# Zhongxu-Wang/ArtSpeech

Measured on AMD Instinct MI355X. Metric: mel frames/sec (whole job; per-GPU = value / n_gpus), acoustic-model inference path, batch 32 x 200-frame utterances, higher is better.
Workload: dtype f32 (f16x3 split-operand MFMA, fp32 accumulate)

## Files before the change

### artspeech_amd/_lib.py

```python
import ctypes
import os

import torch

_HERE = os.path.dirname(os.path.abspath(__file__))
LIB_PATH = os.environ.get("AS_LIB_PATH") or os.path.join(_HERE, "lib", "libartspeech_hip.so")
_lib = None

c_p = ctypes.c_void_p
c_i = ctypes.c_int
c_sz = ctypes.c_size_t
c_f = ctypes.c_float

_SIGNATURES = {
    "as_abi_version": (c_i, []),
    "as_device_status": (c_i, [c_i]),
    "as_device_status_raise_for_test": (c_i, [c_i, c_p]),
    "as_set_range_probe": (c_i, [c_i]),
    "as_prof_enable": (c_i, [c_i]),
    "as_prof_collect": (c_i, [c_p, c_p, c_p, c_p, c_i]),
    "as_prof_hint": (c_i, [ctypes.c_double, ctypes.c_double]),
    "as_prof_bracket_overhead": (c_i, [c_p, c_p]),
    "as_prof_mfma_sustained": (c_i, [c_p, c_p, c_p]),
    "as_mas_workspace_bytes": (c_sz, [c_i, c_i, c_i]),
    "as_mas_f32": (c_i, [c_p, c_p, c_p, c_i, c_i, c_i, c_i, c_p, c_p, c_p, c_p, c_sz, c_p]),
    "as_softmax_mas_f32": (c_i, [c_p, c_p, c_p, c_i, c_i, c_i, c_i, c_i, c_p, c_p, c_p, c_p, c_p, c_sz, c_p]),
}

AS_MAX_TAPS = 25
AS_ABI_VERSION = 10
AS_PROSODY_DIM, AS_PROSODY_TRACKS, AS_PROSODY_DUR, AS_PROSODY_GAIN, AS_PROSODY_OFFSET = 25, 12, 0, 1, 13


class ConvGemmArgs(ctypes.Structure):
    _fields_ = [("Wh", ctypes.c_void_p), ("W", ctypes.c_void_p), ("X", ctypes.c_void_p), ("Xh", ctypes.c_void_p), ("Y", ctypes.c_void_p),
                ("Yh", ctypes.c_void_p), ("bias", ctypes.c_void_p), ("res", ctypes.c_void_p), ("meta", ctypes.c_void_p),
                ("ws", ctypes.c_void_p), ("ws_bytes", ctypes.c_size_t),
                ("M", ctypes.c_int32), ("N", ctypes.c_int32), ("K", ctypes.c_int32), ("T", ctypes.c_int32),
                ("Kp", ctypes.c_int32),
                ("ldx", ctypes.c_int32), ("ldy", ctypes.c_int32), ("ldr", ctypes.c_int32),
                ("act", ctypes.c_int32), ("div_sqrt2", ctypes.c_int32), ("in_act", ctypes.c_int32),
                ("transpose_out", ctypes.c_int32), ("yh_lrelu", ctypes.c_int32), ("n_prod", ctypes.c_int32),
                ("dh", ctypes.c_int32 * AS_MAX_TAPS), ("dw", ctypes.c_int32 * AS_MAX_TAPS),
                ("in_slope", ctypes.c_float), ("act_slope", ctypes.c_float), ("acc_scale", ctypes.c_float),
                ("n_groups", ctypes.c_int32), ("group_cols", ctypes.c_int32), ("range_probe", ctypes.c_int32), ("status", ctypes.c_void_p),
                ("Xh2", ctypes.c_void_p), ("K2", ctypes.c_int32), ("src_col", ctypes.c_void_p), ("N_in", ctypes.c_int32), ("ileave_u", ctypes.c_int32),
                ("slab_tr", ctypes.c_int32), ("n_valid", ctypes.c_void_p)]


_SIGNATURES.update({
    "as_make_meta": (c_i, [c_p, c_p, c_i, c_i, c_i, c_p, c_p]),
    "as_conv_gemm_f32": (c_i, [ctypes.POINTER(ConvGemmArgs), c_p]),
    "as_conv_gemm_workspace_bytes": (c_sz, [ctypes.POINTER(ConvGemmArgs)]),
    "as_conv_gemm_multi_f32": (c_i, [ctypes.POINTER(ConvGemmArgs), c_i, c_p]),
    "as_conv_gemm_multi_tile": (c_i, [ctypes.POINTER(ConvGemmArgs), c_i]),
    "as_conv_gemm_multi_workspace_bytes": (c_sz, [ctypes.POINTER(ConvGemmArgs)]),
    "as_conv_gemm_plan": (c_i, [ctypes.POINTER(ConvGemmArgs), ctypes.POINTER(ctypes.c_int32), ctypes.POINTER(ctypes.c_int32),
                                ctypes.POINTER(ctypes.c_int32)]),
    "as_split_f16x2_bytes": (c_sz, [c_i, c_i]),
    "as_split_f16x2_f32": (c_i, [c_p, c_i, c_i, c_i, c_i, c_f, c_p, c_p]),
    "as_prep_weight_f16x2_bytes": (c_sz, [c_i, c_i, c_i, c_i]),
    "as_prep_weight_f16x2_host": (c_i, [c_p, c_i, c_i, c_i, c_i, c_p, c_p]),
    "as_prep_weight_f16x2_sc_bytes": (c_sz, [c_i, c_i, c_i, c_i, c_i]),
    "as_prep_weight_f16x2_sc_host": (c_i, [c_p, c_p, c_i, c_i, c_i, c_i, c_i, c_p, c_p]),
    "as_embed_groups_f32": (c_i, [c_p, c_i, c_p, c_p, c_i, c_i, c_i, c_i, c_f, c_p, c_i, c_p]),
    "as_channel_layernorm_groups_f32": (c_i, [c_p, c_i, c_i, c_i, c_p, c_p, c_p, c_p, c_i, c_f, c_i, c_p, c_i, c_p]),
    "as_channel_layernorm_split_f32": (c_i, [c_p, c_i, c_i, c_i, c_p, c_p, c_p, c_p, c_i, c_f, c_i, c_p, c_p]),
    "as_relpos_attention_groups_f32": (c_i, [c_p, c_i, c_i, c_i, c_i, c_p, c_p, c_p, c_p, c_i, c_p, c_i, c_i, c_p, c_i, c_p]),
    "as_embed_f32": (c_i, [c_p, c_p, c_i, c_i, c_i, c_f, c_p, c_i, c_p]),
    "as_channel_layernorm_f32": (c_i, [c_p, c_i, c_i, c_i, c_p, c_p, c_f, c_i, c_p, c_i, c_p]),
    "as_adain_f32": (c_i, [c_p, c_i, c_i, c_p, c_i, c_p, c_i, c_p, c_i, c_i, c_p, c_p, c_p, c_i, c_p]),
    "as_adain_split_f32": (c_i, [c_p, c_i, c_i, c_p, c_i, c_p, c_i, c_i, c_i, c_p, c_p]),
    "as_linear_rows_f32": (c_i, [c_p, c_i, c_p, c_p, c_i, c_i, c_i, c_p, c_i, c_p]),
    "as_durations_f32": (c_i, [c_p, c_p, c_p, c_i, c_p, c_p, c_p, c_i, c_p]),
    "as_expand_f32": (c_i, [c_p, c_i, c_i, c_p, c_i, c_i, c_p, c_i, c_p]),
    "as_ref_features_f32": (c_i, [c_p, c_i, c_i, c_p, c_p, c_i, c_i, c_p, c_p, c_i, c_p]),
    "as_crop_f32": (c_i, [c_p, c_i, c_p, c_i, c_p, c_i, c_p, c_i, c_i, c_i, c_p]),
    "as_rows_to_images_f32": (c_i, [c_p, c_i, c_p, c_i, c_i, c_p, c_p, c_i, c_i, c_p]),
    "as_stem_pool_image_f32": (c_i, [c_p, c_p, c_p, c_i, c_p, c_p, c_i, c_i, c_p, c_i, c_p, c_i, c_i, c_i, c_i, c_p, c_i, c_p]),
    "as_dwconv_down_f32": (c_i, [c_p, c_i, c_p, c_p, c_i, c_p, c_i, c_p, c_p, c_i, c_p, c_p, c_i, c_i, c_i, c_i, c_i, c_p]),
    "as_frame_signal_f32": (c_i, [c_p, c_p, c_p, c_i, c_i, c_i, c_i, c_p, c_i, c_p]),
    "as_spec_power_f32": (c_i, [c_p, c_i, c_i, c_i, c_p, c_i, c_p]),
    "as_log_norm_f32": (c_i, [c_p, c_i, c_i, c_i, c_f, c_f, c_f, c_p, c_i, c_p]),
    "as_xl_attention_f32": (c_i, [c_p, c_i, c_i, c_i, c_p, c_i, c_p, c_p, c_f, c_p, c_i, c_i, c_p, c_i, c_p]),
    "as_glu_dwconv_bn_swish_f32": (c_i, [c_p, c_i, c_i, c_p, c_i, c_p, c_p, c_p, c_i, c_p, c_i, c_p]),
    "as_lstm_step0_f32": (c_i, [c_p, c_i, c_i, c_i, c_p, c_i, c_p]),
    "as_bn_lrelu_maxpool_rows_f32": (c_i, [c_p, c_i, c_p, c_i, c_i, c_i, c_i, c_p, c_p, c_f, c_p, c_i, c_i, c_i, c_p]),
    "as_avgpool_down_f32": (c_i, [c_p, c_i, c_p, c_p, c_i, c_p, c_i, c_p, c_p, c_i, c_i, c_p, c_i, c_i, c_i, c_i, c_p]),
    "as_im2col_valid_f32": (c_i, [c_p, c_i, c_p, c_p, c_i, c_p, c_i, c_p, c_p, c_i, c_i, c_i, c_i, c_i, c_i, c_i, c_p]),
    "as_dwconv_down_image_f32": (c_i, [c_p, c_i, c_p, c_p, c_i, c_p, c_p, c_i, c_p, c_p, c_i, c_i, c_i, c_i, c_i, c_p, c_i, c_p]),
    "as_avgpool_down_image_f32": (c_i, [c_p, c_i, c_p, c_p, c_i, c_p, c_i, c_p, c_p, c_i, c_i, c_p, c_i, c_i, c_i, c_i, c_p, c_i, c_i, c_p]),
    "as_im2col_valid_image_f32": (c_i, [c_p, c_i, c_p, c_p, c_p, c_p, c_i, c_i, c_i, c_i, c_i, c_p, c_p]),
    "as_mean_pool_f32": (c_i, [c_p, c_i, c_p, c_i, c_i, c_i, c_p, c_i, c_p]),
    "as_relpos_attention_f32": (c_i, [c_p, c_i, c_i, c_i, c_i, c_p, c_p, c_p, c_i, c_i, c_p, c_i, c_p]),
    "as_relpos_attention_image_f32": (c_i, [c_p, c_i, c_p, c_i, c_i, c_i, c_i, c_p, c_p, c_p, c_p, c_i, c_p, c_i, c_i, c_p, c_i, c_p, c_p]),
    "as_bilstm_f32": (c_i, [c_p, c_i, c_p, c_i, c_i, c_p]),
    "as_bilstm_cluster_bytes": (ctypes.c_size_t, [c_i, c_i]),
    "as_bilstm_cluster_f32": (c_i, [c_p, c_i, c_p, c_i, c_i, c_i, c_p, ctypes.c_size_t, c_p]),
    "as_interleave_phases_f32": (c_i, [c_p, c_i, c_p, c_i, c_i, c_i, c_p, c_i, c_p]),
    "as_mean3_f32": (c_i, [c_p, c_p, c_p, c_i, c_i, c_i, c_p, c_i, c_p]),
})


class LnArgs(ctypes.Structure):
    _fields_ = [("gamma", c_p), ("beta", c_p), ("gamma2", c_p), ("beta2", c_p), ("n_split", ctypes.c_int32), ("eps", ctypes.c_float),
                ("relu", ctypes.c_int32), ("yh", c_p)]


class AdainArgs(ctypes.Structure):
    _fields_ = [("x", c_p), ("ldx", ctypes.c_int32), ("C", ctypes.c_int32), ("gb", c_p), ("gb_off", c_p), ("ldgb", ctypes.c_int32),
                ("gb_sc", ctypes.c_int32), ("col_off", c_p), ("src_off", c_p), ("U", ctypes.c_int32), ("N", ctypes.c_int32),
                ("lrelu", ctypes.c_int32), ("yh", c_p), ("pool_w", c_p), ("pool_b", c_p), ("x_up", c_p), ("ld_up", ctypes.c_int32),
                ("col_w", c_p)]


class DownArgs(ctypes.Structure):
    _fields_ = [("kind", ctypes.c_int32), ("x", c_p), ("ldx", ctypes.c_int32), ("in_off", c_p), ("in_w", c_p), ("Hin", ctypes.c_int32),
                ("y", c_p), ("ldy", ctypes.c_int32), ("out_off", c_p), ("out_w", c_p), ("Hout", ctypes.c_int32), ("w", c_p), ("bias", c_p),
                ("kh", ctypes.c_int32), ("pool_h", ctypes.c_int32), ("Kp", ctypes.c_int32), ("res", c_p), ("ldr", ctypes.c_int32),
                ("B", ctypes.c_int32), ("C", ctypes.c_int32), ("max_out", ctypes.c_int32), ("lrelu", ctypes.c_int32), ("yh", c_p),
                ("n_out", ctypes.c_int32)]


class ResPairArgs(ctypes.Structure):
    _fields_ = [("x", c_p), ("ldx", ctypes.c_int32), ("y", c_p), ("ldy", ctypes.c_int32), ("w1", c_p), ("w2", c_p), ("b1", c_p), ("b2", c_p),
                ("scale1", ctypes.c_float), ("scale2", ctypes.c_float), ("C", ctypes.c_int32), ("N", ctypes.c_int32), ("k", ctypes.c_int32),
                ("dil", ctypes.c_int32), ("slope", ctypes.c_float), ("col_off", c_p), ("B", ctypes.c_int32), ("max_w", ctypes.c_int32),
                ("add1", c_p), ("add2", c_p), ("ld_add", ctypes.c_int32), ("out_div", ctypes.c_float), ("yh", c_p), ("yh_slope", ctypes.c_float),
                ("x_u", ctypes.c_int32), ("x_bias", c_p)]


class ModelCfg(ctypes.Structure):
    _fields_ = [("hidden_dim", ctypes.c_int32), ("dim_in", ctypes.c_int32), ("style_dim", ctypes.c_int32), ("n_mels", ctypes.c_int32),
                ("n_token", ctypes.c_int32), ("reserved", ctypes.c_int32), ("stats", ctypes.c_float * 24)]


class Batch(ctypes.Structure):
    _fields_ = [("B", ctypes.c_int32), ("tok_lens", ctypes.POINTER(ctypes.c_int32)), ("ref_lens", ctypes.POINTER(ctypes.c_int32)),
                ("frames", ctypes.POINTER(ctypes.c_int32))]


class ForwardIO(ctypes.Structure):
    _fields_ = [("tokens", c_p), ("mel", c_p), ("ld_mel", ctypes.c_int32), ("f0_raw", c_p), ("ema_raw", c_p), ("ld_ema", ctypes.c_int32),
                ("forced_dur", c_p), ("mel_out", c_p), ("ld_out", ctypes.c_int32), ("duration", c_p), ("dur_i", c_p), ("frame_off", c_p),
                ("style", c_p), ("feat12", c_p), ("ld_feat", ctypes.c_int32), ("t_en", c_p), ("a_en", c_p), ("ld_en", ctypes.c_int32),
                ("F0", c_p), ("N", c_p), ("EMA", c_p), ("ld_pred", ctypes.c_int32), ("frame_cap", ctypes.c_int32), ("segs", c_p),
                ("voices", c_p), ("ld_voice", ctypes.c_int32), ("n_voices", ctypes.c_int32), ("voice_idx", c_p),
                ("prosody", c_p), ("ld_prosody", ctypes.c_int32)]


class HostIO(ctypes.Structure):
    _fields_ = [("tokens", c_p), ("mel", c_p), ("ld_mel", ctypes.c_int32), ("f0_raw", c_p), ("ema_raw", c_p), ("ld_ema", ctypes.c_int32),
                ("forced_dur", c_p), ("mel_out", c_p), ("ld_out", ctypes.c_int32), ("frame_cap", ctypes.c_int32), ("frame_off", c_p),
                ("voices", c_p), ("ld_voice", ctypes.c_int32), ("n_voices", ctypes.c_int32), ("voice_idx", c_p),
                ("prosody", c_p), ("ld_prosody", ctypes.c_int32)]


class TokenProsody(ctypes.Structure):
    _fields_ = [("rows", c_p), ("ld", ctypes.c_int32), ("smooth", ctypes.c_int32)]


(AS_MOD_FORWARD_A, AS_MOD_FORWARD_B, AS_MOD_ENCODER, AS_MOD_STYLE, AS_MOD_DURATION, AS_MOD_ARTS, AS_MOD_DECODER, AS_MOD_FORWARD_B_CAP,
 AS_MOD_VOICE, AS_MOD_FORWARD_A_VOICE) = range(10)
_pB, _pIO = ctypes.POINTER(Batch), ctypes.POINTER(ForwardIO)
_SIGNATURES.update({
    "as_adain_image_f32": (c_i, [ctypes.POINTER(AdainArgs), c_p]),
    "as_conv_gemm_multi_post_f32": (c_i, [ctypes.POINTER(ConvGemmArgs), ctypes.POINTER(AdainArgs), ctypes.POINTER(ctypes.c_int32),
                                          ctypes.POINTER(LnArgs), c_i, c_p]),
    "as_down_multi_f32": (c_i, [ctypes.POINTER(DownArgs), c_i, c_p]),
    "as_down_strip_rule": (c_i, [c_i, c_i, c_i, c_i, c_i, ctypes.POINTER(ctypes.c_int32), ctypes.POINTER(ctypes.c_int32)]),
    "as_respair_f32": (c_i, [ctypes.POINTER(ResPairArgs), c_p]),
    "as_xl_attention_image_f32": (c_i, [c_p, c_i, c_p, c_p, c_i, c_i, c_i, ctypes.c_float, c_p, c_i, c_i, c_p, c_i, c_p, c_p]),
    "as_mean3_image_f32": (c_i, [c_p, c_p, c_p, c_i, c_i, c_i, ctypes.c_float, c_p, c_p]),
    "as_conv_post_f32": (c_i, [c_p, c_i, c_i, c_i, c_p, c_p, c_i, ctypes.c_float, c_i, c_p, c_p, c_p]),
    "as_rows_image_f32": (c_i, [c_p, c_i, c_i, c_i, c_p, c_p]),
    "as_project_cols_f32": (c_i, [c_p, c_i, c_i, c_i, c_p, c_p, c_i, c_p, c_i, c_p]),
    "as_pointwise_small_f32": (c_i, [c_p, c_i, c_i, c_i, c_p, c_p, c_i, c_p, c_i, c_p, c_p, c_i, c_p, c_p]),
    "as_model_create": (c_i, [c_p, c_sz, ctypes.POINTER(ModelCfg), ctypes.POINTER(c_p)]),
# ... 155 lines not shown
```

### artspeech_amd/csrc/attention.hip

```cpp
#include <cstring>
#include "common.h"
#include "artspeech_hip.h"
#define AS_FILE_CLS AS_CLS_ATTN

#define QT 16
#define KT 64
#define KPAD 65
#define MAXDK 128
#define MAXREL 9

static __device__ __forceinline__ float wmax(float v)
{
#pragma unroll
    for (int o = 32; o > 0; o >>= 1) v = fmaxf(v, __shfl_xor(v, o));
    return v;
}
static __device__ __forceinline__ float wsum(float v)
{
#pragma unroll
    for (int o = 32; o > 0; o >>= 1) v += __shfl_xor(v, o);
    return v;
}

__global__ void __launch_bounds__(256)
// ... 43 lines not shown
    float m[4], l[4], acc[4][2];
#pragma unroll
    for (int qq = 0; qq < 4; ++qq) { m[qq] = -INFINITY; l[qq] = 0.f; acc[qq][0] = 0.f; acc[qq][1] = 0.f; }
    float* Pw = Ps + wave * KT * 4;
    const int d0 = lane, d1 = lane + 64;

    for (int k0 = 0; k0 < N; k0 += KT) {
        __syncthreads();
        for (int i = tid; i < dk * KT; i += 256) {
            const int jj = i % KT, d = i / KT;
            const int kj = k0 + jj;
            const bool ok = kj < N;
            Ks[d * KPAD + jj] = ok ? Kg[(size_t)d * ld + kj] : 0.f;
            Vs[d * KPAD + jj] = ok ? Vg[(size_t)d * ld + kj] : 0.f;
        }
        __syncthreads();
        float s[4] = {0.f, 0.f, 0.f, 0.f};
        const float* qb = Qs + (wave * 4) * dk;
        for (int d = 0; d < dk; ++d) {
            const float kv = Ks[d * KPAD + lane];
#pragma unroll
            for (int qq = 0; qq < 4; ++qq) s[qq] += qb[qq * dk + d] * kv;
        }
        const int kj = k0 + lane;
#pragma unroll
        for (int qq = 0; qq < 4; ++qq) {
            const int qi = q0 + wave * 4 + qq;
            float sc = s[qq] / scale;
            const int r = kj - qi + window;
            if (r >= 0 && r < nrel) sc += Rk[(wave * 4 + qq) * MAXREL + r];
            if (kj >= N) sc = -INFINITY;
            const float mn = fmaxf(m[qq], wmax(sc));
            const float p = (kj < N) ? expf(sc - mn) : 0.f;
            const float corr = expf(m[qq] - mn);
            l[qq] = l[qq] * corr + wsum(p);
            acc[qq][0] *= corr;
            acc[qq][1] *= corr;
            m[qq] = mn;
            Pw[lane * 4 + qq] = p;
        }
        __syncthreads();
        const int jn = (N - k0) < KT ? (N - k0) : KT;
        if (d0 < dk) {
            const bool two = d1 < dk;
            for (int jj = 0; jj < jn; ++jj) {
                const float4 p4 = *reinterpret_cast<const float4*>(Pw + jj * 4);
                const float v0 = Vs[d0 * KPAD + jj];
                const float v1 = two ? Vs[d1 * KPAD + jj] : 0.f;
                acc[0][0] += p4.x * v0; acc[1][0] += p4.y * v0; acc[2][0] += p4.z * v0; acc[3][0] += p4.w * v0;
                acc[0][1] += p4.x * v1; acc[1][1] += p4.y * v1; acc[2][1] += p4.z * v1; acc[3][1] += p4.w * v1;
            }
#pragma unroll
            for (int qq = 0; qq < 4; ++qq) {
                const int qi = q0 + wave * 4 + qq;
                for (int r = 0; r < nrel; ++r) {
                    const int jg = qi + r - window;
                    if (jg < k0 || jg >= k0 + jn || jg < 0) continue;
                    const float p = Pw[(jg - k0) * 4 + qq];
                    acc[qq][0] += p * Ev[r * dk + d0];
                    if (two) acc[qq][1] += p * Ev[r * dk + d1];
                }
            }
        }
    }
    __syncthreads();
    float* Os = Ks;
    if (d0 < dk) {
#pragma unroll
        for (int qq = 0; qq < 4; ++qq) {
            Os[d0 * QT + wave * 4 + qq] = acc[qq][0] / l[qq];
            if (d1 < dk) Os[d1 * QT + wave * 4 + qq] = acc[qq][1] / l[qq];
        }
    }
    __syncthreads();
    for (int i = tid; i < dk * QT; i += 256) {
        const int q = i % QT, d = i / QT;
        if (q0 + q < N) out[(size_t)(h * dk + d) * ldo + o0 + q0 + q] = Os[d * QT + q];
    }
}

#include "conv_gemm.h"
#define FK 64
typedef __attribute__((address_space(3))) void attn_lds_void;
struct AttnImageArgs {
    const float* qkv;
    const uint16_t* qkv_h;
    const float *ek1, *ev1, *ek2, *ev2;
    const int* col_off;
    float* out;
    uint16_t* out_h;
    int ld, C, window, b_split, n_total, ldo;
};

template <int NW>
__global__ void __launch_bounds__(NW * 64)
relpos_attention_image_kernel(const AttnImageArgs a)
{
    constexpr int DK = 128, KB = DK / 16, NT = NW * 64, NQ = NW * 32;
    const int grp = a.ek2 ? (int)blockIdx.z / a.b_split : 0;
    const float* emb_k = a.ek1 + (ptrdiff_t)grp * (a.ek2 - a.ek1);
    const float* emb_v = a.ev1 + (ptrdiff_t)grp * (a.ev2 - a.ev1);
    extern __shared__ __attribute__((aligned(16))) unsigned char smraw[];
    u32x4_t* Kt = reinterpret_cast<u32x4_t*>(smraw);
    u32x4_t* Vt = Kt + 2 * (2 * KB * 2 * FK);
    u32x4_t* EkI = Vt + 2 * 4 * 2 * DK;
    u32x4_t* EvT = EkI + 2 * KB * 2 * 32;
    float* Rk = reinterpret_cast<float*>(EvT + 2 * 2 * DK);
    float* Pb = Rk + NQ * MAXREL;

    const int b = blockIdx.z, h = blockIdx.y;
    const int o0 = a.col_off[b], N = a.col_off[b + 1] - o0;
    const int q0 = blockIdx.x * NQ;
    const int tid = threadIdx.x, lane = tid & 63, wave = __builtin_amdgcn_readfirstlane(tid >> 6), g = lane >> 5, lq = lane & 31;
    const int nrel = 2 * a.window + 1, window = a.window;
    const size_t NX = (size_t)a.n_total + 1;
    if (a.out_h && blockIdx.x == 0 && b == 0 && tid < KB * 4) {
        reinterpret_cast<u32x4_t*>(a.out_h)[((size_t)(h * KB) * 4 + tid) * NX + a.n_total] = u32x4_t{0u, 0u, 0u, 0u};
    }
    if (q0 >= N) return;
    const float cs = 1.44269504088896340736f / sqrtf((float)DK);
    const u32x4_t* img = reinterpret_cast<const u32x4_t*>(a.qkv_h);
    const int qkb0 = (h * DK) / 16, kkb0 = (a.C + h * DK) / 16;
    const float* Vg = a.qkv + (size_t)(2 * a.C + h * DK) * a.ld + o0;

    const int ql = wave * 32 + lq, qi = q0 + ql, qw0 = q0 + wave * 32;
    const size_t qcol = (size_t)min(o0 + qi, a.n_total);
    u32x4_t Qh[KB], Ql[KB];
#pragma unroll
    for (int kb = 0; kb < KB; ++kb) {
        Qh[kb] = img[((size_t)(qkb0 + kb) * 4 + g) * NX + qcol];
        Ql[kb] = img[((size_t)(qkb0 + kb) * 4 + 2 + g) * NX + qcol];
    }
    const __amdgpu_buffer_rsrc_t rsK = __builtin_amdgcn_make_buffer_rsrc(const_cast<uint16_t*>(a.qkv_h), 0,
                                                                         (int)((unsigned)(3 * a.C / 16) * 4u * (unsigned)NX * 16u), 0x00020000);
    (void)rsK;
    (void)kkb0;
    auto issue_k = [&](int k0, int buf) {
#if __HIP_DEVICE_COMPILE__
#pragma unroll
        for (int i = 0; i < 2 * KB * 2 / NW; ++i) {
            const int ch = wave + NW * i, pp = ch / (KB * 2), kb = (ch / 2) % KB, gg = ch & 1;
            const unsigned voff = (unsigned)((((kkb0 + kb) * 4 + pp * 2 + gg) * NX + (size_t)(o0 + k0 + lane)) * 16u);
            __builtin_amdgcn_raw_ptr_buffer_load_lds(rsK, (attn_lds_void*)(smraw + (size_t)buf * (2 * KB * 2 * FK * 16) + ch * (FK * 16)), 16, voff, 0,
                                                     0, 0);
        }
#endif
    };
    constexpr int VI = DK * (FK / 4) / NT;
    float vr[VI][4];
    auto load_v = [&](int k0) {
#pragma unroll
        for (int it = 0; it < VI; ++it) {
            const int idx = tid + it * NT, kq = idx % (FK / 4), d = idx / (FK / 4), kk = k0 + kq * 4;
            const float* row = Vg + (size_t)d * a.ld;
            if (o0 + k0 + FK + 3 < a.ld) {
                const f32x4 v4 = *reinterpret_cast<const f32x4 __attribute__((aligned(4)))*>(row + kk);
                vr[it][0] = v4[0]; vr[it][1] = v4[1]; vr[it][2] = v4[2]; vr[it][3] = v4[3];
            } else {
#pragma unroll
                for (int e = 0; e < 4; ++e) vr[it][e] = row[min(kk + e, N - 1)];
            }
        }
    };
    auto store_v = [&](int k0) {
        u32x2_t* V2 = reinterpret_cast<u32x2_t*>(Vt);
#pragma unroll
        for (int it = 0; it < VI; ++it) {
            const int idx = tid + it * NT, kq = idx % (FK / 4), d = idx / (FK / 4);
            const int kk = kq * 4, sb = kk >> 5, w32 = kk & 31, ig = w32 >> 3, gg = (w32 & 7) >> 2, c = sb * 2 + (ig >> 1);
            float v[4];
#pragma unroll
            for (int e = 0; e < 4; ++e) v[e] = k0 + kk + e < N ? vr[it][e] : 0.f;
            unsigned h0, l0, h1, l1;
            split2_pair(v[0], v[1], h0, l0);
            split2_pair(v[2], v[3], h1, l1);
            const u32x2_t hh = {h0, h1}, ll = {l0, l1};
            V2[(((0 * 4 + c) * 2 + gg) * DK + d) * 2 + (ig & 1)] = hh;
            V2[(((1 * 4 + c) * 2 + gg) * DK + d) * 2 + (ig & 1)] = ll;
        }
    };
    issue_k(0, 0);
    load_v(0);
    {
        constexpr int EI = 32 * (DK / 8) / NT, VI2 = 2 * DK / NT;
        typedef f32x4 __attribute__((aligned(4))) f32x4u;
        f32x4 xe[EI][2];
        float xv[VI2][8];
#pragma unroll
        for (int it = 0; it < EI; ++it) {
            const int idx = tid + it * NT, r = idx & 31, dg = idx >> 5;
            const int rc = r < nrel ? r : 0;
            xe[it][0] = *reinterpret_cast<const f32x4u*>(emb_k + rc * DK + dg * 8);
            xe[it][1] = *reinterpret_cast<const f32x4u*>(emb_k + rc * DK + dg * 8 + 4);
        }
#pragma unroll
        for (int it = 0; it < VI2; ++it) {
            const int idx = tid + it * NT, d = idx % DK, gg = idx / DK;
#pragma unroll
            for (int j = 0; j < 8; ++j) xv[it][j] = emb_v[min(8 * gg + j, nrel - 1) * DK + d];
        }
#pragma unroll
        for (int it = 0; it < EI; ++it) {
            const int idx = tid + it * NT, r = idx & 31, dg = idx >> 5;
            float x[8];
#pragma unroll
            for (int j = 0; j < 8; ++j) x[j] = r < nrel ? xe[it][j >> 2][j & 3] : 0.f;
            u32x4_t hh, ll;
            split2(x, hh, ll);
            EkI[((0 * KB + (dg >> 1)) * 2 + (dg & 1)) * 32 + r] = hh;
            EkI[((1 * KB + (dg >> 1)) * 2 + (dg & 1)) * 32 + r] = ll;
        }
#pragma unroll
        for (int it = 0; it < VI2; ++it) {
            const int idx = tid + it * NT, d = idx % DK, gg = idx / DK;
            float x[8];
#pragma unroll
            for (int j = 0; j < 8; ++j) x[j] = 8 * gg + j < nrel ? xv[it][j] : 0.f;
            u32x4_t hh, ll;
            split2(x, hh, ll);
            EvT[(0 * 2 + gg) * DK + d] = hh;
            EvT[(1 * 2 + gg) * DK + d] = ll;
        }
    }
    __syncthreads();
    {
        f32x16 SR;
#pragma unroll
        for (int e = 0; e < 16; ++e) SR[e] = 0.f;
#pragma unroll
        for (int kb = 0; kb < KB; ++kb) {
            const f16x8 ah = __builtin_bit_cast(f16x8, EkI[((0 * KB + kb) * 2 + g) * 32 + lq]);
            const f16x8 al = __builtin_bit_cast(f16x8, EkI[((1 * KB + kb) * 2 + g) * 32 + lq]);
            SR = __builtin_amdgcn_mfma_f32_32x32x16_f16(ah, __builtin_bit_cast(f16x8, Ql[kb]), SR, 0, 0, 0);
            SR = __builtin_amdgcn_mfma_f32_32x32x16_f16(al, __builtin_bit_cast(f16x8, Qh[kb]), SR, 0, 0, 0);
            SR = __builtin_amdgcn_mfma_f32_32x32x16_f16(ah, __builtin_bit_cast(f16x8, Qh[kb]), SR, 0, 0, 0);
        }
#pragma unroll
        for (int e = 0; e < 8; ++e) {
            const int r = 8 * (e >> 2) + 4 * g + (e & 3);
            if (r < nrel) Rk[ql * MAXREL + r] = SR[e] * cs;
        }
    }
    float m = -INFINITY, lsum = 0.f;
    f32x16 acc[4];
#pragma unroll
    for (int mb = 0; mb < 4; ++mb)
#pragma unroll
        for (int e = 0; e < 16; ++e) acc[mb][e] = 0.f;

    int buf = 0;
    for (int k0 = 0; k0 < N; k0 += FK, buf ^= 1) {
        store_v(k0);
        asm volatile("s_waitcnt vmcnt(0)" ::: "memory");
        __syncthreads();
        if (k0 + FK < N) {
            issue_k(k0 + FK, buf ^ 1);
            load_v(k0 + FK);
        }
        const u32x4_t* Kc = Kt + (size_t)buf * (2 * KB * 2 * FK);
        f32x16 S[2];
#pragma unroll
        for (int sb = 0; sb < 2; ++sb) {
#pragma unroll
            for (int e = 0; e < 16; ++e) S[sb][e] = 0.f;
#pragma unroll
            for (int kb = 0; kb < KB; ++kb) {
                const f16x8 ah = __builtin_bit_cast(f16x8, Kc[(0 * KB * 2 + kb * 2 + g) * FK + sb * 32 + lq]);
                const f16x8 al = __builtin_bit_cast(f16x8, Kc[(1 * KB * 2 + kb * 2 + g) * FK + sb * 32 + lq]);
                S[sb] = __builtin_amdgcn_mfma_f32_32x32x16_f16(ah, __builtin_bit_cast(f16x8, Ql[kb]), S[sb], 0, 0, 0);
                S[sb] = __builtin_amdgcn_mfma_f32_32x32x16_f16(al, __builtin_bit_cast(f16x8, Qh[kb]), S[sb], 0, 0, 0);
                S[sb] = __builtin_amdgcn_mfma_f32_32x32x16_f16(ah, __builtin_bit_cast(f16x8, Qh[kb]), S[sb], 0, 0, 0);
            }
        }
        bool band[2];
        float mx = -INFINITY;
#pragma unroll
        for (int sb = 0; sb < 2; ++sb) {
            const int kb0 = k0 + sb * 32;
            band[sb] = kb0 <= qw0 + 31 + window && kb0 + 31 >= qw0 - window;
#pragma unroll
            for (int e = 0; e < 16; ++e) {
                const int key = kb0 + 8 * (e >> 2) + 4 * g + (e & 3);
                float sc = S[sb][e] * cs;
                if (band[sb]) {
                    const int r = key - qi + window;
                    if (r >= 0 && r < nrel) sc += Rk[ql * MAXREL + r];
                }
                if (key >= N) sc = -INFINITY;
                S[sb][e] = sc;
                mx = fmaxf(mx, sc);
            }
        }
        mx = fmaxf(mx, __shfl_xor(mx, 32));
        const float mn = fmaxf(m, mx);
        const float corr = __builtin_amdgcn_exp2f(m - mn);
        m = mn;
        lsum *= corr;
#pragma unroll
        for (int mb = 0; mb < 4; ++mb)
#pragma unroll
            for (int e = 0; e < 16; ++e) acc[mb][e] *= corr;
#pragma unroll
        for (int sb = 0; sb < 2; ++sb)
#pragma unroll
            for (int e = 0; e < 16; ++e) {
                const float pe = __builtin_amdgcn_exp2f(S[sb][e] - mn);
                S[sb][e] = pe;
                lsum += pe;
            }
#pragma unroll
        for (int sb = 0; sb < 2; ++sb) {
            if (!band[sb]) continue;
            const int kb0 = k0 + sb * 32;
            if (g == 0) {
#pragma unroll
                for (int e4 = 0; e4 < 4; ++e4) *reinterpret_cast<f32x4*>(Pb + ql * 16 + e4 * 4) = f32x4{0.f, 0.f, 0.f, 0.f};
            }
            __builtin_amdgcn_wave_barrier();
#pragma unroll
            for (int e = 0; e < 16; ++e) {
                const int r = kb0 + 8 * (e >> 2) + 4 * g + (e & 3) - qi + window;
                if (r >= 0 && r < nrel) Pb[ql * 16 + r] = S[sb][e];
            }
            __builtin_amdgcn_wave_barrier();
            float pb[8];
            {
                const f32x4 p0 = *reinterpret_cast<const f32x4*>(Pb + ql * 16 + 8 * g), p1 = *reinterpret_cast<const f32x4*>(Pb + ql * 16 + 8 * g + 4);
#pragma unroll
                for (int e = 0; e < 4; ++e) { pb[e] = p0[e]; pb[4 + e] = p1[e]; }
            }
            u32x4_t bh, bl;
            split2(pb, bh, bl);
#pragma unroll
            for (int mb = 0; mb < 4; ++mb) {
                const f16x8 eh = __builtin_bit_cast(f16x8, EvT[(0 * 2 + g) * DK + mb * 32 + lq]);
                const f16x8 el = __builtin_bit_cast(f16x8, EvT[(1 * 2 + g) * DK + mb * 32 + lq]);
                acc[mb] = __builtin_amdgcn_mfma_f32_32x32x16_f16(eh, __builtin_bit_cast(f16x8, bl), acc[mb], 0, 0, 0);
                acc[mb] = __builtin_amdgcn_mfma_f32_32x32x16_f16(el, __builtin_bit_cast(f16x8, bh), acc[mb], 0, 0, 0);
                acc[mb] = __builtin_amdgcn_mfma_f32_32x32x16_f16(eh, __builtin_bit_cast(f16x8, bh), acc[mb], 0, 0, 0);
            }
            __builtin_amdgcn_wave_barrier();
        }
#pragma unroll
        for (int c = 0; c < 4; ++c) {
            float pv[8];
#pragma unroll
            for (int j = 0; j < 8; ++j) pv[j] = S[c >> 1][(c & 1) * 8 + j];
            u32x4_t ph, pl;
            split2(pv, ph, pl);
#pragma unroll
            for (int mb = 0; mb < 4; ++mb) {
                const f16x8 vh = __builtin_bit_cast(f16x8, Vt[((0 * 4 + c) * 2 + g) * DK + mb * 32 + lq]);
                const f16x8 vl = __builtin_bit_cast(f16x8, Vt[((1 * 4 + c) * 2 + g) * DK + mb * 32 + lq]);
                acc[mb] = __builtin_amdgcn_mfma_f32_32x32x16_f16(vh, __builtin_bit_cast(f16x8, pl), acc[mb], 0, 0, 0);
                acc[mb] = __builtin_amdgcn_mfma_f32_32x32x16_f16(vl, __builtin_bit_cast(f16x8, ph), acc[mb], 0, 0, 0);
                acc[mb] = __builtin_amdgcn_mfma_f32_32x32x16_f16(vh, __builtin_bit_cast(f16x8, ph), acc[mb], 0, 0, 0);
            }
        }
        __syncthreads();
    }
    const float ltot = lsum + __shfl_xor(lsum, 32);
    if (qi < N) {
        const float inv = 1.0f / ltot;
#pragma unroll
        for (int mb = 0; mb < 4; ++mb)
#pragma unroll
            for (int e4 = 0; e4 < 4; ++e4) {
                float v[4];
#pragma unroll
                for (int e = 0; e < 4; ++e) v[e] = acc[mb][e4 * 4 + e] * inv;
                const int d = mb * 32 + 8 * e4 + 4 * g;
                if (a.out) {
#pragma unroll
                    for (int e = 0; e < 4; ++e) a.out[(size_t)(h * DK + d + e) * a.ldo + o0 + qi] = v[e];
                }
                if (a.out_h) {
                    unsigned h0, l0, h1, l1;
                    split2_pair(v[0], v[1], h0, l0);
                    split2_pair(v[2], v[3], h1, l1);
                    const size_t kbo = (size_t)(h * KB + mb * 2 + (e4 >> 1));
                    u32x2_t* oh = reinterpret_cast<u32x2_t*>(a.out_h);
                    oh[((kbo * 4 + (e4 & 1)) * NX + o0 + qi) * 2 + g] = u32x2_t{h0, h1};
                    oh[((kbo * 4 + 2 + (e4 & 1)) * NX + o0 + qi) * 2 + g] = u32x2_t{l0, l1};
                }
            }
    }
}

template <int NW>
static int launch_attention_image(const AttnImageArgs& a, int heads, int B, int max_len, hipStream_t stream)
{
    constexpr int NQ = NW * 32;
    const size_t smem = (size_t)(2 * (2 * 8 * 2 * FK) + 2 * 4 * 2 * 128 + 2 * 8 * 2 * 32 + 2 * 2 * 128) * 16 + sizeof(float) * (NQ * MAXREL + NQ * 16);
    AS_LDS_OPT_IN(relpos_attention_image_kernel<NW>, 160 * 1024);
    AsProfScope prof__(AS_FILE_CLS, 0, 0, stream);
    hipLaunchKernelGGL(relpos_attention_image_kernel<NW>, dim3(as_cdiv(max_len, NQ), heads, B), dim3(NW * 64), smem, stream, a);
    AS_CHECK_LAUNCH();
    return AS_OK;
}

extern "C" int as_relpos_attention_image_f32(const float* qkv, int ld, const uint16_t* qkv_h, int n_total, int C, int heads, int window,
                                             const float* emb_rel_k, const float* emb_rel_v, const float* emb_rel_k2, const float* emb_rel_v2,
                                             int b_split, const int32_t* col_off, int B, int max_len, float* out, int ldo, uint16_t* out_h,
                                             as_stream_t stream)
{
    if ((emb_rel_k2 == nullptr) != (emb_rel_v2 == nullptr) || (emb_rel_k2 && b_split <= 0)) return AS_EINVAL;
    if (!qkv || !qkv_h || !emb_rel_k || !emb_rel_v || !col_off || (!out && !out_h) || C <= 0 || heads <= 0 || C % heads || n_total < 0 ||
        ld < n_total || (out && ldo < n_total))
        return AS_EINVAL;
    if (C / heads != 128 || 2 * window + 1 > MAXREL || window < 0 || B < 0) return AS_EINVAL;
    if (((reinterpret_cast<uintptr_t>(qkv_h) | reinterpret_cast<uintptr_t>(out_h)) & 15) != 0) return AS_EINVAL;
    if ((double)(3 * C / 16) * 64.0 * (n_total + 1.0) >= 2147483648.0) return AS_EINVAL;
    if (B == 0 || max_len <= 0) return AS_OK;
    AttnImageArgs a;
    a.qkv = qkv; a.qkv_h = qkv_h; a.ek1 = emb_rel_k; a.ev1 = emb_rel_v; a.ek2 = emb_rel_k2; a.ev2 = emb_rel_v2; a.col_off = col_off;
    a.out = out; a.out_h = out_h; a.ld = ld; a.C = C; a.window = window; a.b_split = b_split; a.n_total = n_total; a.ldo = ldo;
    if (max_len <= 64) return launch_attention_image<2>(a, heads, B, max_len, (hipStream_t)stream);
    return launch_attention_image<4>(a, heads, B, max_len, (hipStream_t)stream);
}

extern "C" int as_relpos_attention_groups_f32(const float* qkv, int ld, int C, int heads, int window, const float* emb_rel_k,
                                              const float* emb_rel_v, const float* emb_rel_k2, const float* emb_rel_v2, int b_split,
                                              const int32_t* col_off, int B, int max_len, float* out, int ldo, as_stream_t stream)
{
    if ((emb_rel_k2 == nullptr) != (emb_rel_v2 == nullptr) || (emb_rel_k2 && b_split <= 0)) return AS_EINVAL;
    if (!qkv || !emb_rel_k || !emb_rel_v || !col_off || !out || C <= 0 || heads <= 0 || C % heads) return AS_EINVAL;
    const int dk = C / heads;
    if (dk > MAXDK || 2 * window + 1 > MAXREL || window < 0 || B < 0) return AS_EINVAL;
    if (B == 0 || max_len <= 0) return AS_OK;
    const size_t smem = sizeof(float) * ((size_t)2 * dk * KPAD + QT * dk + 4 * KT * 4 + QT * MAXREL + 2 * MAXREL * dk);
    AS_LDS_OPT_IN(relpos_attention_kernel, 160 * 1024);
    AsProfScope prof__(AS_FILE_CLS, 0, 0, (hipStream_t)stream);
    hipLaunchKernelGGL(relpos_attention_kernel, dim3(as_cdiv(max_len, QT), heads, B), dim3(256), smem, (hipStream_t)stream,
                       qkv, ld, C, heads, window, emb_rel_k, emb_rel_v, emb_rel_k2, emb_rel_v2, b_split, col_off, out, ldo);
    AS_CHECK_LAUNCH();
    return AS_OK;
}

extern "C" int as_relpos_attention_f32(const float* qkv, int ld, int C, int heads, int window, const float* emb_rel_k,
                                       const float* emb_rel_v, const int32_t* col_off, int B, int max_len, float* out,
                                       int ldo, as_stream_t stream)
{
    return as_relpos_attention_groups_f32(qkv, ld, C, heads, window, emb_rel_k, emb_rel_v, nullptr, nullptr, 0, col_off, B, max_len, out,
                                          ldo, stream);
}
```

### include/artspeech_hip.h

```cpp
#ifndef ARTSPEECH_HIP_H
#define ARTSPEECH_HIP_H
#include <stddef.h>
#include <stdint.h>
#ifdef __cplusplus
extern "C" {
#endif

typedef void* as_stream_t;

#define AS_ABI_VERSION 10
int as_abi_version(void);

#define AS_EDEVICE (-3)
enum { AS_STATUS_LSTM_TIMEOUT = 0, AS_STATUS_MAS_TIMEOUT = 1, AS_STATUS_BAD_TOKEN = 2, AS_STATUS_F16_RANGE = 3, AS_STATUS_BAD_LAYOUT = 4,
       AS_STATUS_CAPACITY = 5, AS_STATUS_BAD_VOICE = 6, AS_STATUS_KINDS = 7 };
int as_device_status(int clear);
int as_device_status_raise_for_test(int kind, as_stream_t stream);
int as_set_range_probe(int on);
#define AS_PROBE_THIS 2

int as_prof_enable(int on);
int as_prof_collect(double* ms, double* flops, double* bytes, int32_t* launches, int n_classes);
int as_prof_hint(double flops, double bytes);
int as_prof_bracket_overhead(as_stream_t stream, double* overhead_ms);
// ... 8 lines not shown
                       size_t workspace_bytes, as_stream_t stream);

#define AS_META_MAX_H 1023
#define AS_META_MAX_W 4194303
#define AS_META_PACK(h, w, H, W) \
    ((uint64_t)(h) | ((uint64_t)(H) << 10) | ((uint64_t)(w) << 20) | ((uint64_t)(W) << 42))
#define AS_META_h(md) ((int)((md) & 1023u))
#define AS_META_H(md) ((int)(((md) >> 10) & 1023u))
#define AS_META_w(md) ((int)(((md) >> 20) & 4194303u))
#define AS_META_W(md) ((int)((md) >> 42))
int as_make_meta(const int32_t* widths, const int32_t* col_off, int B, int H, int n_cols_max,
                 uint64_t* meta, as_stream_t stream);

#define AS_MAX_TAPS 25
typedef struct ConvGemmArgs {
    const uint16_t* Wh;
    const float* W;
    const float* X;
    const uint16_t* Xh;
    float* Y;
    uint16_t* Yh;
    const float* bias;
    const float* res;
    const uint64_t* meta;
    void* ws;
    size_t ws_bytes;
    int32_t M, N, K, T;
    int32_t Kp;
    int32_t ldx, ldy, ldr;
    int32_t act;
    int32_t div_sqrt2;
    int32_t in_act;
    int32_t transpose_out;
    int32_t yh_lrelu;
    int32_t n_prod;
    int32_t dh[AS_MAX_TAPS];
    int32_t dw[AS_MAX_TAPS];
    float in_slope, act_slope;
    float acc_scale;
    int32_t n_groups, group_cols;
    int32_t range_probe;
    uint32_t* status;
    const uint16_t* Xh2;
    int32_t K2;
    const int32_t* src_col;
    int32_t N_in;
    int32_t ileave_u;
    int32_t slab_tr;
    const int32_t* n_valid;
} ConvGemmArgs;
#define AS_SLOPE_PATH 0.2f
int as_conv_gemm_f32(const ConvGemmArgs* args_host, as_stream_t stream);
#define AS_MAX_MULTI 6
int as_conv_gemm_multi_f32(const ConvGemmArgs* list_host, int n, as_stream_t stream);
int as_conv_gemm_multi_tile(const ConvGemmArgs* list_host, int n);
size_t as_conv_gemm_multi_workspace_bytes(const ConvGemmArgs* args_host);
int as_conv_gemm_plan(const ConvGemmArgs* args_host, int32_t* kind, int32_t* tile, int32_t* slices);
size_t as_conv_gemm_workspace_bytes(const ConvGemmArgs* args_host);
size_t as_split_f16x2_bytes(int K, int N);
int as_split_f16x2_f32(const float* x, int ldx, int K, int N, int in_act, float in_slope, uint16_t* xh, as_stream_t stream);
int as_split_f16x2_cap_f32(const float* x, int ldx, int K, int N, const int32_t* n_valid, int in_act, float in_slope, uint16_t* xh,
                           as_stream_t stream);
size_t as_prep_weight_f16x2_bytes(int G, int Cout, int Cin, int T);
int as_prep_weight_f16x2_host(const float* w_host, int G, int Cout, int Cin, int T, uint16_t* wh_host, float* scale_out);
size_t as_prep_weight_f16x2_sc_bytes(int G, int Cout, int Cin, int T, int Cin2);
int as_prep_weight_f16x2_sc_host(const float* w_host, const float* w2_host, int G, int Cout, int Cin, int T, int Cin2, uint16_t* wh_host,
                                 float* scale_out);

int as_embed_f32(const int32_t* tokens, const float* emb, int C, int N, int V, float scale, float* y, int ldy,
                 as_stream_t stream);
int as_embed_groups_f32(const int32_t* tokens, int n_tok, const float* emb, const float* emb2, int n_split, int C, int N, int V,
                        float scale, float* y, int ldy, as_stream_t stream);
int as_channel_layernorm_groups_f32(const float* x, int ldx, int C, int N, const float* gamma, const float* beta, const float* gamma2,
                                    const float* beta2, int n_split, float eps, int relu, float* y, int ldy, as_stream_t stream);
int as_channel_layernorm_split_f32(const float* x, int ldx, int C, int N, const float* gamma, const float* beta, const float* gamma2,
                                   const float* beta2, int n_split, float eps, int relu, uint16_t* xs, as_stream_t stream);
int as_relpos_attention_groups_f32(const float* qkv, int ld, int C, int heads, int window, const float* emb_rel_k,
                                   const float* emb_rel_v, const float* emb_rel_k2, const float* emb_rel_v2, int b_split,
                                   const int32_t* col_off, int B, int max_len, float* out, int ldo, as_stream_t stream);
int as_relpos_attention_image_f32(const float* qkv, int ld, const uint16_t* qkv_h, int n_total, int C, int heads, int window,
                                  const float* emb_rel_k, const float* emb_rel_v, const float* emb_rel_k2, const float* emb_rel_v2,
                                  int b_split, const int32_t* col_off, int B, int max_len, float* out, int ldo, uint16_t* out_h,
                                  as_stream_t stream);
int as_channel_layernorm_f32(const float* x, int ldx, int C, int N, const float* gamma, const float* beta, float eps,
                             int relu, float* y, int ldy, as_stream_t stream);
int as_adain_f32(const float* x, int ldx, int C, const float* gamma_beta, int ldgb, const int32_t* col_off, int B,
                 float* y, int ldy, int lrelu, const float* pool_w, const float* pool_b, float* x_up, int ld_up,
                 as_stream_t stream);
int as_adain_split_f32(const float* x, int ldx, int C, const float* gamma_beta, int ldgb, const int32_t* col_off, int B, int N,
                       int lrelu, uint16_t* xs, as_stream_t stream);
typedef struct AsAdainArgs {
    const float* x;
    int32_t ldx, C;
    const float* gb;
    const int32_t* gb_off;
    int32_t ldgb, gb_sc;
    const int32_t* col_off;
    const int32_t* src_off;
    int32_t U, N;
    int32_t lrelu;
    uint16_t* yh;
    const float* pool_w;
    const float* pool_b;
    float* x_up;
    int32_t ld_up;
    const int32_t* col_w;
} AsAdainArgs;
int as_adain_image_f32(const AsAdainArgs* args_host, as_stream_t stream);
typedef struct AsLnArgs {
    const float *gamma, *beta, *gamma2, *beta2;
    int32_t n_split;
    float eps;
    int32_t relu;
    uint16_t* yh;
} AsLnArgs;
int as_conv_gemm_multi_post_f32(const ConvGemmArgs* list_host, const AsAdainArgs* post_host, const int32_t* post_max_w,
                                const AsLnArgs* post_ln_host, int n, as_stream_t stream);
int as_rows_image_f32(const float* x, int ldx, int K, int B, uint16_t* xh, as_stream_t stream);
int as_project_cols_f32(const float* x, int ldx, int K, int N, const float* w, const float* bias, int M, float* y, int ldy,
                        as_stream_t stream);
int as_pointwise_small_f32(const float* x, int ldx, int K, int N, const float* w, const float* bias, int M, float* y1, int ld1,
                           uint16_t* yh1, float* y2, int ld2, uint16_t* yh2, as_stream_t stream);
int as_linear_rows_f32(const float* x, int ldx, const float* w, const float* bias, int B, int M, int K, float* y,
                       int ldy, as_stream_t stream);
int as_durations_f32(const float* dur_f32, const int32_t* forced_dur, const int32_t* tok_off, int B, int32_t* dur_i32,
                     int32_t* frame_off, int32_t* tok_of_frame, int max_frames, as_stream_t stream);
int as_expand_f32(const float* x, int ldx, int C, const int32_t* tok_of_frame, int n_frames, int repeat, float* y,
                  int ldy, as_stream_t stream);
int as_ref_features_f32(const float* mel, int ldm, int n_mels, const float* f0_raw, const float* ema_raw, int lde,
                        int N, const float* stats24, float* feat, int ldf, as_stream_t stream);
int as_crop_f32(const float* src, int lds, const int32_t* src_off, int start, float* dst, int ldd,
                const int32_t* dst_off, int B, int C, int max_len, as_stream_t stream);
int as_rows_to_images_f32(const float* src, int lds, const int32_t* src_off, int start, int H, float* dst,
                          const int32_t* img_off, int B, int max_w, as_stream_t stream);
int as_dwconv_down_f32(const float* x, int ldx, const int32_t* in_off, const int32_t* in_w, int Hin, float* y, int ldy,
                       const int32_t* out_off, const int32_t* out_w, int Hout, const float* w, const float* bias,
                       int kh, int B, int C, int max_out, int lrelu, as_stream_t stream);
int as_bn_lrelu_maxpool_rows_f32(const float* x, int ldx, const int32_t* tok_off, int B, int C, int H, int k, const float* scale,
                                 const float* shift, float slope, float* y, int ldy, int to_channels, int total_frames,
                                 as_stream_t stream);
int as_avgpool_down_f32(const float* x, int ldx, const int32_t* in_off, const int32_t* in_w, int Hin, float* y, int ldy,
                        const int32_t* out_off, const int32_t* out_w, int Hout, int pool_h, const float* res, int ldr,
                        int B, int C, int max_out, as_stream_t stream);
int as_im2col_valid_f32(const float* x, int ldx, const int32_t* in_off, const int32_t* in_w, int Hin, float* col,
                        int ldc, const int32_t* out_off, const int32_t* out_w, int Hout, int K, int stride, int lrelu,
                        int B, int C, int max_out, as_stream_t stream);
int as_dwconv_down_image_f32(const float* x, int ldx, const int32_t* in_off, const int32_t* in_w, int Hin, const int32_t* out_off,
                             const int32_t* out_w, int Hout, const float* w, const float* bias, int kh, int B, int C, int max_out,
                             int lrelu, uint16_t* yh, int n_out, as_stream_t stream);
int as_avgpool_down_image_f32(const float* x, int ldx, const int32_t* in_off, const int32_t* in_w, int Hin, float* y, int ldy,
                              const int32_t* out_off, const int32_t* out_w, int Hout, int pool_h, const float* res, int ldr, int B,
                              int C, int max_out, uint16_t* yh, int n_out, int yh_lrelu, as_stream_t stream);
int as_stem_pool_image_f32(const float* x, const int32_t* in_off, const int32_t* in_w, int Hin, const int32_t* out_off,
                           const int32_t* out_w, int Hout, int pool_h, const float* w, int Kp, const float* bias, int kh, int B, int C,
                           int max_out, uint16_t* yh, int n_out, as_stream_t stream);
typedef struct AsDownArgs {
    int32_t kind;
    const float* x; int32_t ldx;
    const int32_t* in_off; const int32_t* in_w; int32_t Hin;
    float* y; int32_t ldy;
    const int32_t* out_off; const int32_t* out_w; int32_t Hout;
    const float* w; const float* bias;
    int32_t kh, pool_h, Kp;
    const float* res; int32_t ldr;
    int32_t B, C, max_out, lrelu;
    uint16_t* yh; int32_t n_out;
// ... 248 lines not shown
```

Baseline: 1.751 million.

## Add single-tile relpos attention variant with register-held K and smaller LDS

For sequences no longer than one key tile (max_len <= 64), adds a template variant that holds K fragments in registers instead of staging them through double-buffered LDS. It shrinks the relative-embedding LDS area to MAXREL rows, drops the K/V pipelining loop, and allows two or three workgroups per CU. Q loads are reordered to overlap with V loads, and the second K sub-block is prefetched inside the MFMA loop. The cost is more register pressure from keeping the K arrays live, and a code path that only matters when utterances are short.

New measurement: 1.776 million, median of 6. +1.4%, better.

```diff
diff --git a/artspeech_amd/_lib.py b/artspeech_amd/_lib.py
--- a/artspeech_amd/_lib.py
+++ b/artspeech_amd/_lib.py
@@ -94,6 +94,7 @@
     "as_mean_pool_f32": (c_i, [c_p, c_i, c_p, c_i, c_i, c_i, c_p, c_i, c_p]),
     "as_relpos_attention_f32": (c_i, [c_p, c_i, c_i, c_i, c_i, c_p, c_p, c_p, c_i, c_i, c_p, c_i, c_p]),
     "as_relpos_attention_image_f32": (c_i, [c_p, c_i, c_p, c_i, c_i, c_i, c_i, c_p, c_p, c_p, c_p, c_i, c_p, c_i, c_i, c_p, c_i, c_p, c_p]),
+    "as_relpos_attention_image_lds_bytes": (c_i, [c_i]),
     "as_bilstm_f32": (c_i, [c_p, c_i, c_p, c_i, c_i, c_p]),
     "as_bilstm_cluster_bytes": (ctypes.c_size_t, [c_i, c_i]),
     "as_bilstm_cluster_f32": (c_i, [c_p, c_i, c_p, c_i, c_i, c_i, c_p, ctypes.c_size_t, c_p]),
diff --git a/artspeech_amd/csrc/attention.hip b/artspeech_amd/csrc/attention.hip
--- a/artspeech_amd/csrc/attention.hip
+++ b/artspeech_amd/csrc/attention.hip
@@ -149,6 +149,11 @@
 #include "conv_gemm.h"
 #define FK 64
 typedef __attribute__((address_space(3))) void attn_lds_void;
+static constexpr size_t attn_image_lds_bytes(int nw, bool one)
+{
+    return (size_t)((one ? 0 : 2 * (2 * 8 * 2 * FK)) + 2 * 4 * 2 * 128 + 2 * 8 * 2 * (one ? MAXREL : 32) + 2 * 2 * 128) * 16 +
+           sizeof(float) * (nw * 32 * MAXREL + nw * 32 * 16);
+}
 struct AttnImageArgs {
     const float* qkv;
     const uint16_t* qkv_h;
@@ -159,19 +164,20 @@
     int ld, C, window, b_split, n_total, ldo;
 };
 
-template <int NW>
-__global__ void __launch_bounds__(NW * 64)
+template <int NW, bool ONE>
+__global__ void __launch_bounds__(NW * 64, ONE ? 2 : 1)
 relpos_attention_image_kernel(const AttnImageArgs a)
 {
     constexpr int DK = 128, KB = DK / 16, NT = NW * 64, NQ = NW * 32;
+    constexpr int ER = ONE ? MAXREL : 32;
     const int grp = a.ek2 ? (int)blockIdx.z / a.b_split : 0;
     const float* emb_k = a.ek1 + (ptrdiff_t)grp * (a.ek2 - a.ek1);
     const float* emb_v = a.ev1 + (ptrdiff_t)grp * (a.ev2 - a.ev1);
     extern __shared__ __attribute__((aligned(16))) unsigned char smraw[];
     u32x4_t* Kt = reinterpret_cast<u32x4_t*>(smraw);
-    u32x4_t* Vt = Kt + 2 * (2 * KB * 2 * FK);
+    u32x4_t* Vt = Kt + (ONE ? 0 : 2 * (2 * KB * 2 * FK));
     u32x4_t* EkI = Vt + 2 * 4 * 2 * DK;
-    u32x4_t* EvT = EkI + 2 * KB * 2 * 32;
+    u32x4_t* EvT = EkI + 2 * KB * 2 * ER;
     float* Rk = reinterpret_cast<float*>(EvT + 2 * 2 * DK);
     float* Pb = Rk + NQ * MAXREL;
 
@@ -193,11 +199,19 @@
     const int ql = wave * 32 + lq, qi = q0 + ql, qw0 = q0 + wave * 32;
     const size_t qcol = (size_t)min(o0 + qi, a.n_total);
     u32x4_t Qh[KB], Ql[KB];
-#pragma unroll
-    for (int kb = 0; kb < KB; ++kb) {
-        Qh[kb] = img[((size_t)(qkb0 + kb) * 4 + g) * NX + qcol];
-        Ql[kb] = img[((size_t)(qkb0 + kb) * 4 + 2 + g) * NX + qcol];
-    }
+    if constexpr (!ONE) {
+#pragma unroll
+        for (int kb = 0; kb < KB; ++kb) {
+            Qh[kb] = img[((size_t)(qkb0 + kb) * 4 + g) * NX + qcol];
+            Ql[kb] = img[((size_t)(qkb0 + kb) * 4 + 2 + g) * NX + qcol];
+        }
+    }
+    u32x4_t Kh[2][KB], Kl[2][KB];
+    auto load_k = [&](int sb, int kb) {
+        const size_t kcol = (size_t)min(o0 + sb * 32 + lq, a.n_total);
+        Kh[sb][kb] = img[((size_t)(kkb0 + kb) * 4 + g) * NX + kcol];
+        Kl[sb][kb] = img[((size_t)(kkb0 + kb) * 4 + 2 + g) * NX + kcol];
+    };
     const __amdgpu_buffer_rsrc_t rsK = __builtin_amdgcn_make_buffer_rsrc(const_cast<uint16_t*>(a.qkv_h), 0,
                                                                          (int)((unsigned)(3 * a.C / 16) * 4u * (unsigned)NX * 16u), 0x00020000);
     (void)rsK;
@@ -216,17 +230,29 @@
     constexpr int VI = DK * (FK / 4) / NT;
     float vr[VI][4];
     auto load_v = [&](int k0) {
-#pragma unroll
-        for (int it = 0; it < VI; ++it) {
+        const bool quads = o0 + k0 + FK + 3 < a.ld;
+        auto item = [&](int it, bool q4) {
             const int idx = tid + it * NT, kq = idx % (FK / 4), d = idx / (FK / 4), kk = k0 + kq * 4;
             const float* row = Vg + (size_t)d * a.ld;
-            if (o0 + k0 + FK + 3 < a.ld) {
+            if (q4) {
                 const f32x4 v4 = *reinterpret_cast<const f32x4 __attribute__((aligned(4)))*>(row + kk);
                 vr[it][0] = v4[0]; vr[it][1] = v4[1]; vr[it][2] = v4[2]; vr[it][3] = v4[3];
             } else {
 #pragma unroll
                 for (int e = 0; e < 4; ++e) vr[it][e] = row[min(kk + e, N - 1)];
             }
+        };
+        if constexpr (ONE) {
+            if (quads) {
+#pragma unroll
+                for (int it = 0; it < VI; ++it) item(it, true);
+            } else {
+#pragma unroll
+                for (int it = 0; it < VI; ++it) item(it, false);
+            }
+        } else {
+#pragma unroll
+            for (int it = 0; it < VI; ++it) item(it, quads);
         }
     };
     auto store_v = [&](int k0) {
@@ -246,16 +272,23 @@
             V2[(((1 * 4 + c) * 2 + gg) * DK + d) * 2 + (ig & 1)] = ll;
         }
     };
-    issue_k(0, 0);
+    if constexpr (!ONE) issue_k(0, 0);
     load_v(0);
+    if constexpr (ONE) {
+#pragma unroll
+        for (int kb = 0; kb < KB; ++kb) {
+            Qh[kb] = img[((size_t)(qkb0 + kb) * 4 + g) * NX + qcol];
+            Ql[kb] = img[((size_t)(qkb0 + kb) * 4 + 2 + g) * NX + qcol];
+        }
+    }
     {
-        constexpr int EI = 32 * (DK / 8) / NT, VI2 = 2 * DK / NT;
+        constexpr int EI = (ER * (DK / 8) + NT - 1) / NT, VI2 = 2 * DK / NT;
         typedef f32x4 __attribute__((aligned(4))) f32x4u;
         f32x4 xe[EI][2];
         float xv[VI2][8];
 #pragma unroll
         for (int it = 0; it < EI; ++it) {
-            const int idx = tid + it * NT, r = idx & 31, dg = idx >> 5;
+            const int idx = tid + it * NT, r = ONE ? idx / (DK / 8) : idx & 31, dg = ONE ? idx % (DK / 8) : idx >> 5;
             const int rc = r < nrel ? r : 0;
             xe[it][0] = *reinterpret_cast<const f32x4u*>(emb_k + rc * DK + dg * 8);
             xe[it][1] = *reinterpret_cast<const f32x4u*>(emb_k + rc * DK + dg * 8 + 4);
@@ -268,14 +301,16 @@
         }
 #pragma unroll
         for (int it = 0; it < EI; ++it) {
-            const int idx = tid + it * NT, r = idx & 31, dg = idx >> 5;
+            const int idx = tid + it * NT, r = ONE ? idx / (DK / 8) : idx & 31, dg = ONE ? idx % (DK / 8) : idx >> 5;
             float x[8];
 #pragma unroll
             for (int j = 0; j < 8; ++j) x[j] = r < nrel ? xe[it][j >> 2][j & 3] : 0.f;
             u32x4_t hh, ll;
             split2(x, hh, ll);
-            EkI[((0 * KB + (dg >> 1)) * 2 + (dg & 1)) * 32 + r] = hh;
-            EkI[((1 * KB + (dg >> 1)) * 2 + (dg & 1)) * 32 + r] = ll;
+            if (!ONE || r < nrel) {
+                EkI[((0 * KB + (dg >> 1)) * 2 + (dg & 1)) * ER + r] = hh;
+                EkI[((1 * KB + (dg >> 1)) * 2 + (dg & 1)) * ER + r] = ll;
+            }
         }
 #pragma unroll
         for (int it = 0; it < VI2; ++it) {
@@ -289,6 +324,11 @@
             EvT[(1 * 2 + gg) * DK + d] = ll;
         }
     }
+    if constexpr (ONE) {
+        store_v(0);
+#pragma unroll
+        for (int kb = 0; kb < KB; ++kb) load_k(0, kb);
+    }
     __syncthreads();
     {
         f32x16 SR;
@@ -296,8 +336,10 @@
         for (int e = 0; e < 16; ++e) SR[e] = 0.f;
 #pragma unroll
         for (int kb = 0; kb < KB; ++kb) {
-            const f16x8 ah = __builtin_bit_cast(f16x8, EkI[((0 * KB + kb) * 2 + g) * 32 + lq]);
-            const f16x8 al = __builtin_bit_cast(f16x8, EkI[((1 * KB + kb) * 2 + g) * 32 + lq]);
+            const int er = ONE && lq >= nrel ? 0 : lq;
+            u32x4_t eh = EkI[((0 * KB + kb) * 2 + g) * ER + er], el = EkI[((1 * KB + kb) * 2 + g) * ER + er];
+            if (ONE && lq >= nrel) eh = el = u32x4_t{0u, 0u, 0u, 0u};
+            const f16x8 ah = __builtin_bit_cast(f16x8, eh), al = __builtin_bit_cast(f16x8, el);
             SR = __builtin_amdgcn_mfma_f32_32x32x16_f16(ah, __builtin_bit_cast(f16x8, Ql[kb]), SR, 0, 0, 0);
             SR = __builtin_amdgcn_mfma_f32_32x32x16_f16(al, __builtin_bit_cast(f16x8, Qh[kb]), SR, 0, 0, 0);
             SR = __builtin_amdgcn_mfma_f32_32x32x16_f16(ah, __builtin_bit_cast(f16x8, Qh[kb]), SR, 0, 0, 0);
@@ -307,6 +349,7 @@
             const int r = 8 * (e >> 2) + 4 * g + (e & 3);
             if (r < nrel) Rk[ql * MAXREL + r] = SR[e] * cs;
         }
+        if constexpr (ONE) __builtin_amdgcn_wave_barrier();
     }
     float m = -INFINITY, lsum = 0.f;
     f32x16 acc[4];
@@ -317,12 +360,14 @@
 
     int buf = 0;
     for (int k0 = 0; k0 < N; k0 += FK, buf ^= 1) {
-        store_v(k0);
-        asm volatile("s_waitcnt vmcnt(0)" ::: "memory");
-        __syncthreads();
-        if (k0 + FK < N) {
-            issue_k(k0 + FK, buf ^ 1);
-            load_v(k0 + FK);
+        if constexpr (!ONE) {
+            store_v(k0);
+            asm volatile("s_waitcnt vmcnt(0)" ::: "memory");
+            __syncthreads();
+            if (k0 + FK < N) {
+                issue_k(k0 + FK, buf ^ 1);
+                load_v(k0 + FK);
+            }
         }
         const u32x4_t* Kc = Kt + (size_t)buf * (2 * KB * 2 * FK);
         f32x16 S[2];
@@ -332,11 +377,17 @@
             for (int e = 0; e < 16; ++e) S[sb][e] = 0.f;
 #pragma unroll
             for (int kb = 0; kb < KB; ++kb) {
-                const f16x8 ah = __builtin_bit_cast(f16x8, Kc[(0 * KB * 2 + kb * 2 + g) * FK + sb * 32 + lq]);
-                const f16x8 al = __builtin_bit_cast(f16x8, Kc[(1 * KB * 2 + kb * 2 + g) * FK + sb * 32 + lq]);
+                const f16x8 ah = __builtin_bit_cast(f16x8, ONE ? Kh[sb][kb] : Kc[(0 * KB * 2 + kb * 2 + g) * FK + sb * 32 + lq]);
+                const f16x8 al = __builtin_bit_cast(f16x8, ONE ? Kl[sb][kb] : Kc[(1 * KB * 2 + kb * 2 + g) * FK + sb * 32 + lq]);
                 S[sb] = __builtin_amdgcn_mfma_f32_32x32x16_f16(ah, __builtin_bit_cast(f16x8, Ql[kb]), S[sb], 0, 0, 0);
                 S[sb] = __builtin_amdgcn_mfma_f32_32x32x16_f16(al, __builtin_bit_cast(f16x8, Qh[kb]), S[sb], 0, 0, 0);
                 S[sb] = __builtin_amdgcn_mfma_f32_32x32x16_f16(ah, __builtin_bit_cast(f16x8, Qh[kb]), S[sb], 0, 0, 0);
+                if constexpr (ONE) {
+                    if (sb == 0) {
+                        load_k(1, kb);
+                        __builtin_amdgcn_sched_barrier(0);
+                    }
+                }
             }
         }
         bool band[2];
@@ -424,6 +475,7 @@
                 acc[mb] = __builtin_amdgcn_mfma_f32_32x32x16_f16(vh, __builtin_bit_cast(f16x8, ph), acc[mb], 0, 0, 0);
             }
         }
+        if constexpr (ONE) break;
         __syncthreads();
     }
     const float ltot = lsum + __shfl_xor(lsum, 32);
@@ -454,14 +506,15 @@
     }
 }
 
-template <int NW>
+template <int NW, bool ONE>
 static int launch_attention_image(const AttnImageArgs& a, int heads, int B, int max_len, hipStream_t stream)
 {
     constexpr int NQ = NW * 32;
-    const size_t smem = (size_t)(2 * (2 * 8 * 2 * FK) + 2 * 4 * 2 * 128 + 2 * 8 * 2 * 32 + 2 * 2 * 128) * 16 + sizeof(float) * (NQ * MAXREL + NQ * 16);
-    AS_LDS_OPT_IN(relpos_attention_image_kernel<NW>, 160 * 1024);
+    constexpr size_t smem = attn_image_lds_bytes(NW, ONE);
+    static_assert(!ONE || 3 * smem <= 160 * 1024, "three short-sequence workgroups share a CU's LDS");
+    if constexpr (smem > 64 * 1024) AS_LDS_OPT_IN((relpos_attention_image_kernel<NW, ONE>), 160 * 1024);
     AsProfScope prof__(AS_FILE_CLS, 0, 0, stream);
-    hipLaunchKernelGGL(relpos_attention_image_kernel<NW>, dim3(as_cdiv(max_len, NQ), heads, B), dim3(NW * 64), smem, stream, a);
+    hipLaunchKernelGGL((relpos_attention_image_kernel<NW, ONE>), dim3(as_cdiv(max_len, NQ), heads, B), dim3(NW * 64), smem, stream, a);
     AS_CHECK_LAUNCH();
     return AS_OK;
 }
@@ -482,8 +535,14 @@
     AttnImageArgs a;
     a.qkv = qkv; a.qkv_h = qkv_h; a.ek1 = emb_rel_k; a.ev1 = emb_rel_v; a.ek2 = emb_rel_k2; a.ev2 = emb_rel_v2; a.col_off = col_off;
     a.out = out; a.out_h = out_h; a.ld = ld; a.C = C; a.window = window; a.b_split = b_split; a.n_total = n_total; a.ldo = ldo;
-    if (max_len <= 64) return launch_attention_image<2>(a, heads, B, max_len, (hipStream_t)stream);
-    return launch_attention_image<4>(a, heads, B, max_len, (hipStream_t)stream);
+    if (max_len <= FK) return launch_attention_image<2, true>(a, heads, B, max_len, (hipStream_t)stream);
+    return launch_attention_image<4, false>(a, heads, B, max_len, (hipStream_t)stream);
+}
+
+extern "C" int as_relpos_attention_image_lds_bytes(int max_len)
+{
+    if (max_len <= 0) return 0;
+    return (int)(max_len <= FK ? attn_image_lds_bytes(2, true) : attn_image_lds_bytes(4, false));
 }
 
 extern "C" int as_relpos_attention_groups_f32(const float* qkv, int ld, int C, int heads, int window, const float* emb_rel_k,
diff --git a/include/artspeech_hip.h b/include/artspeech_hip.h
--- a/include/artspeech_hip.h
+++ b/include/artspeech_hip.h
@@ -114,6 +114,7 @@
                                   const float* emb_rel_k, const float* emb_rel_v, const float* emb_rel_k2, const float* emb_rel_v2,
                                   int b_split, const int32_t* col_off, int B, int max_len, float* out, int ldo, uint16_t* out_h,
                                   as_stream_t stream);
+int as_relpos_attention_image_lds_bytes(int max_len);
 int as_channel_layernorm_f32(const float* x, int ldx, int C, int N, const float* gamma, const float* beta, float eps,
                              int relu, float* y, int ldy, as_stream_t stream);
 int as_adain_f32(const float* x, int ldx, int C, const float* gamma_beta, int ldgb, const int32_t* col_off, int B,
```
